# dotnetpower/infomesh

Measured on AMD Instinct MI355X. Metric: queries/sec (hybrid BM25+dense search, 1.25M docs), higher is better.
Workload: dtype bf16; 1 GPU; model=bge-small-en(random-init) encoder + BM25 CSR + cosine top-k, global_batch=128, seq_len=32, parallelism=shard1, mode=hybrid, docs_per_gpu=1250000, total_docs=1250000

## Files before the change

infomesh_amd/models/bert.py:

```python
from __future__ import annotations

from dataclasses import dataclass

import torch

from ..ops import kernels as K
from ..ops import reference as R


@dataclass(frozen=True)
class BertConfig:
    vocab_size: int
    hidden: int
    layers: int
    heads: int
    ffn: int
    max_pos: int = 512
    eps: float = 1e-12

    @property
    def head_dim(self) -> int:
        return self.hidden // self.heads


# ... 6 lines not shown

    def w(*shape, s=std):
        return torch.randn(*shape, generator=g) * s

    ws: dict[str, torch.Tensor] = {
        "embed.word": w(cfg.vocab_size, H),
        "embed.pos": w(cfg.max_pos, H),
        "embed.ln.g": torch.ones(H),
        "embed.ln.b": torch.zeros(H),
    }
    for i in range(cfg.layers):
        p = f"layer.{i}."
        ws[p + "qkv.w"] = w(3 * H, H)
        ws[p + "qkv.b"] = torch.zeros(3 * H)
        ws[p + "attn_out.w"] = w(H, H)
        ws[p + "attn_out.b"] = torch.zeros(H)
        ws[p + "ln1.g"] = torch.ones(H)
        ws[p + "ln1.b"] = torch.zeros(H)
        ws[p + "ffn_in.w"] = w(F, H)
        ws[p + "ffn_in.b"] = torch.zeros(F)
        ws[p + "ffn_out.w"] = w(H, F)
        ws[p + "ffn_out.b"] = torch.zeros(H)
        ws[p + "ln2.g"] = torch.ones(H)
        ws[p + "ln2.b"] = torch.zeros(H)
    out = {}
    for k, v in ws.items():
        t = v.to(device)
        out[k] = t if k.endswith(".b") and "ln" not in k else t.to(dtype)
        if "ln" in k:
            out[k] = t.to(dtype)
    return out


class BertEncoder:
    def __init__(self, cfg: BertConfig, weights: dict[str, torch.Tensor],
                 use_fused_attn: bool = True):
        self.cfg = cfg
        self.w = weights
        self.use_fused_attn = use_fused_attn and cfg.head_dim in (32, 64,
                                                                  96, 128)

    def forward(self, ids: torch.Tensor, lens: torch.Tensor) -> torch.Tensor:
        cfg, w = self.cfg, self.w
        B, S = ids.shape
        if S % 32 != 0:
            pad = 32 - S % 32
            ids = torch.nn.functional.pad(ids, (0, pad))
            S += pad
        H, nh, d = cfg.hidden, cfg.heads, cfg.head_dim
        pos_ids = torch.arange(S, device=ids.device, dtype=torch.int32)\
            .repeat(B)
        x = K.gather(w["embed.word"], ids.reshape(-1))
        x = K.add(x, K.gather(w["embed.pos"], pos_ids))
        x = K.layernorm(x, w["embed.ln.g"], w["embed.ln.b"], eps=cfg.eps)

        vl = lens.repeat_interleave(nh).contiguous()
        scale = d ** -0.5
        vl_b = lens.contiguous()
        for i in range(cfg.layers):
            p = f"layer.{i}."
            qkv = K.gemm_nt(x, w[p + "qkv.w"], bias=w[p + "qkv.b"])
            if self.use_fused_attn:
                qkv5 = qkv.view(B, S, 3, nh, d)
                qv = qkv5[:, :, 0].permute(0, 2, 1, 3)
                kv = qkv5[:, :, 1].permute(0, 2, 1, 3)
                vv = qkv5[:, :, 2].permute(0, 2, 1, 3)
                ctx = K.attn_fused(qv, kv, vv, valid_len=vl_b, scale=scale)
            else:
                q, k, vt = K.qkv_split(qkv, B, S, nh, nh, d)
                scores = K.gemm_nt(q, k, out_f32=True, alpha=scale)
                probs = K.softmax(scores, valid_len=vl)
                ctx = K.gemm_nt(probs, vt)
            merged = K.merge_heads(ctx, B, S, nh, d)
            attn = K.gemm_nt(merged, w[p + "attn_out.w"],
                             bias=w[p + "attn_out.b"])
            x = K.layernorm(attn, w[p + "ln1.g"], w[p + "ln1.b"],
                            residual=x, eps=cfg.eps)
            h = K.gemm_nt(x, w[p + "ffn_in.w"], bias=w[p + "ffn_in.b"],
                          act="gelu")
            o = K.gemm_nt(h, w[p + "ffn_out.w"], bias=w[p + "ffn_out.b"])
            x = K.layernorm(o, w[p + "ln2.g"], w[p + "ln2.b"],
                            residual=x, eps=cfg.eps)
        return x.view(B, S, H)

    def forward_reference(self, ids: torch.Tensor,
                          lens: torch.Tensor) -> torch.Tensor:
        cfg = self.cfg
        w = {k: v.float().cpu() for k, v in self.w.items()}
        B, S = ids.shape
        H, nh, d = cfg.hidden, cfg.heads, cfg.head_dim
        ids_l = ids.cpu().long()
        x = w["embed.word"][ids_l] + w["embed.pos"][:S].unsqueeze(0)
        x = R.layernorm(x, w["embed.ln.g"], w["embed.ln.b"], eps=cfg.eps)
        vl = lens.cpu().repeat_interleave(nh)
        for i in range(cfg.layers):
            p = f"layer.{i}."
            qkv = R.gemm_nt(x.view(B * S, H), w[p + "qkv.w"], w[p + "qkv.b"])
            qkv = qkv.view(B, S, 3, nh, d)
            q = qkv[:, :, 0].permute(0, 2, 1, 3).reshape(B * nh, S, d)
            k = qkv[:, :, 1].permute(0, 2, 1, 3).reshape(B * nh, S, d)
            v = qkv[:, :, 2].permute(0, 2, 1, 3).reshape(B * nh, S, d)
            scores = torch.matmul(q, k.transpose(1, 2)) * d ** -0.5
            probs = R.softmax(scores, valid_len=vl)
            ctx = torch.matmul(probs, v)
            merged = ctx.view(B, nh, S, d).permute(0, 2, 1, 3).reshape(B * S, H)
            attn = R.gemm_nt(merged, w[p + "attn_out.w"], w[p + "attn_out.b"])
            x = R.layernorm(attn, w[p + "ln1.g"], w[p + "ln1.b"],
                            residual=x.view(B * S, H), eps=cfg.eps)
            h = R.gemm_nt(x, w[p + "ffn_in.w"], w[p + "ffn_in.b"], act="gelu")
            o = R.gemm_nt(h, w[p + "ffn_out.w"], w[p + "ffn_out.b"])
            x = R.layernorm(o, w[p + "ln2.g"], w[p + "ln2.b"],
                            residual=x, eps=cfg.eps)
        return x.view(B, S, H)
```

infomesh_amd/models/encoder.py:

```python
from __future__ import annotations

import torch

from ..ops import kernels as K
from ..ops import reference as R
from .bert import BertConfig, BertEncoder, init_bert_weights
from .tokenizer import HashTokenizer

BGE_SMALL = BertConfig(vocab_size=30522, hidden=384, layers=12, heads=12,
                       ffn=1536, max_pos=512)

EMBED_DIM = BGE_SMALL.hidden


class EmbeddingEncoder:

    def __init__(self, device: str = "cuda", seed: int = 1234,
                 cfg: BertConfig = BGE_SMALL, max_len: int = 128,
                 use_graph: bool = True):
        self.cfg = cfg
        self.device = device
        self.max_len = max_len
        self.tokenizer = HashTokenizer(cfg.vocab_size)
        self.bert = BertEncoder(cfg, init_bert_weights(cfg, seed, device))
        from ..ops.graphs import GraphedCallable
        self._graphed = GraphedCallable(self._encode_impl, enabled=use_graph)

    def _encode_impl(self, ids: torch.Tensor,
                     lens: torch.Tensor) -> torch.Tensor:
        hidden = self.bert.forward(ids, lens)
        return K.pool(hidden, lens, mode="cls", l2=True)

    def encode_ids(self, ids: torch.Tensor, lens: torch.Tensor) -> torch.Tensor:
        return self._graphed(ids, lens)

    def encode_texts(self, texts: list[str]) -> torch.Tensor:
        ids_l, lens = self.tokenizer.encode_batch(texts, self.max_len)
        ids = torch.tensor(ids_l, dtype=torch.int32, device=self.device)
        lens_t = torch.tensor(lens, dtype=torch.int32, device=self.device)
        return self.encode_ids(ids, lens_t)

    def encode_ids_reference(self, ids: torch.Tensor,
                             lens: torch.Tensor) -> torch.Tensor:
        hidden = self.bert.forward_reference(ids, lens)
        return R.pool(hidden.bfloat16(), lens.cpu(), mode="cls", l2=True)
```

infomesh_amd/ops/_ext.py:

```python
from __future__ import annotations

import ctypes
from ctypes import c_float, c_int, c_long, c_void_p
from pathlib import Path

from ..errors import GpuExtensionMissing

_LIB: ctypes.CDLL | None = None
_LOAD_ERROR: str | None = None

_SIGNATURES: dict[str, list] = {
    "infomesh_gemm_bf16_nt": [c_void_p, c_void_p, c_void_p, c_void_p,
                              c_int, c_int, c_int, c_int,
                              c_long, c_long, c_long,
                              c_int, c_float, c_int, c_void_p],
    "infomesh_layernorm": [c_void_p, c_void_p, c_void_p, c_void_p,
                           c_void_p, c_void_p, c_long, c_int, c_float,
                           c_void_p],
    "infomesh_rmsnorm": [c_void_p, c_void_p, c_void_p, c_void_p,
                         c_void_p, c_long, c_int, c_float, c_void_p],
    "infomesh_softmax": [c_void_p, c_void_p, c_void_p, c_long, c_int,
                         c_int, c_int, c_float, c_void_p],
    "infomesh_bias_act": [c_void_p, c_void_p, c_long, c_int, c_int, c_void_p],
    "infomesh_silu_mul": [c_void_p, c_void_p, c_void_p, c_long, c_void_p],
    "infomesh_add": [c_void_p, c_void_p, c_void_p, c_long, c_void_p],
    "infomesh_rope": [c_void_p, c_void_p, c_void_p, c_void_p, c_long,
                      c_int, c_int, c_int, c_void_p],
    "infomesh_gather": [c_void_p, c_void_p, c_void_p, c_long, c_int,
                        c_float, c_void_p],
    "infomesh_pool": [c_void_p, c_void_p, c_void_p, c_int, c_int, c_int,
                      c_int, c_int, c_void_p],
    "infomesh_argmax": [c_void_p, c_void_p, c_long, c_int, c_void_p],
    "infomesh_topk": [c_void_p, c_void_p, c_void_p, c_void_p, c_int,
                      c_long, c_int, c_void_p, c_void_p],
    "infomesh_topk_masked": [c_void_p, c_void_p, c_void_p, c_void_p, c_int,
                             c_long, c_int, c_void_p, c_void_p, c_long,
                             c_void_p],
    "infomesh_filter_bitmask": [c_void_p, c_void_p, c_void_p, c_long,
                                c_int, c_void_p],
    "infomesh_filter_bitmask_sets": [c_void_p, c_void_p, c_void_p, c_void_p,
                                     c_void_p, c_long, c_int, c_void_p],
    "infomesh_term_bitmask": [c_void_p, c_long, c_void_p, c_void_p,
                              c_void_p, c_void_p, c_int, c_void_p, c_int,
                              c_long, c_long, c_long, c_long, c_void_p],
    "infomesh_term_block_docs": [],
    "infomesh_topk_workspace_u32": [c_int],
    "infomesh_topk_zero_u32": [c_int],
    "infomesh_bm25_block": [c_void_p, c_void_p, c_void_p, c_void_p,
                            c_void_p, c_void_p, c_void_p, c_void_p,
                            c_void_p, c_void_p, c_int, c_int, c_long,
                            c_long, c_long, c_int, c_float, c_float,
                            c_float, c_void_p],
    "infomesh_score_combine": [c_void_p, c_void_p, c_void_p, c_float,
                               c_float, c_long, c_void_p],
    "infomesh_simhash_fingerprint": [c_void_p, c_void_p, c_void_p, c_long,
                                     c_void_p],
    "infomesh_hamming_scan": [c_void_p, c_void_p, c_void_p, c_void_p,
                              c_void_p, c_void_p, c_int, c_long, c_int,
                              c_int, c_void_p],
    "infomesh_attn_decode": [c_void_p, c_void_p, c_void_p, c_void_p,
                             c_void_p, c_int, c_int, c_int, c_int, c_int,
                             c_float, c_void_p],
    "infomesh_attn_decode_split": [c_void_p, c_void_p, c_void_p, c_void_p,
                                   c_void_p, c_void_p, c_int, c_int, c_int,
                                   c_int, c_int, c_int, c_float, c_void_p],
    "infomesh_attn_fused": [c_void_p, c_void_p, c_void_p, c_void_p,
                            c_void_p, c_int, c_int, c_int, c_int, c_int,
                            c_int, c_long, c_long, c_long, c_long, c_long,
                            c_long, c_long, c_long, c_long,
                            c_int, c_float, c_void_p],
    "infomesh_kv_append": [c_void_p, c_void_p, c_void_p, c_void_p,
                           c_void_p, c_int, c_int, c_int, c_int, c_void_p],
    "infomesh_dense_scores": [c_void_p, c_void_p, c_void_p,
                              c_int, c_long, c_int, c_float, c_void_p],
    "infomesh_dense_scores_fp8": [c_void_p, c_void_p, c_void_p,
                                  c_int, c_long, c_int, c_float,
                                  c_void_p],
    "infomesh_gemm8_bf16_nt": [c_void_p, c_void_p, c_void_p, c_void_p,
                               c_int, c_int, c_int, c_int,
                               c_long, c_long, c_long,
                               c_int, c_float, c_int, c_void_p],
    "infomesh_gemv_bf16_nt": [c_void_p, c_void_p, c_void_p, c_void_p,
                              c_int, c_int, c_int, c_int,
                              c_long, c_long, c_long,
                              c_int, c_float, c_int, c_void_p],
    "infomesh_qkv_split": [c_void_p, c_void_p, c_void_p, c_void_p,
                           c_void_p, c_void_p, c_void_p,
                           c_int, c_int, c_int, c_int, c_int, c_int,
                           c_void_p],
    "infomesh_merge_heads": [c_void_p, c_void_p, c_int, c_int, c_int,
                             c_int, c_void_p],
    "infomesh_silu_mul_fused": [c_void_p, c_void_p, c_long, c_int,
                                c_void_p],
    "infomesh_gemm_tile": [c_int, c_int, c_int, c_int],
    "infomesh_gemm_bmax_width": [c_int, c_int, c_int, c_int],
    "infomesh_gemm_bf16_nt_bmax": [c_void_p, c_void_p, c_void_p, c_void_p,
                                   c_void_p, c_int, c_int, c_int, c_int,
                                   c_long, c_long, c_long,
                                   c_int, c_float, c_void_p],
    "infomesh_topk_pruned": [c_void_p, c_void_p, c_int, c_void_p, c_void_p,
                             c_void_p, c_int, c_long, c_int, c_void_p],
    "infomesh_topk_pruned_workspace_u32": [c_int, c_long, c_int, c_int],
    "infomesh_topk_pruned_zero_u32": [c_int],
# ... 13 lines not shown
    "infomesh_domtop_chunk_docs": [],
    "infomesh_domtop_lds_slots": [],
    "infomesh_domtop_k_max": [],
    "infomesh_domain_best": [c_void_p, c_void_p, c_void_p, c_void_p,
                             c_void_p, c_void_p, c_int, c_int, c_long,
                             c_long, c_int, c_int, c_int, c_int, c_void_p],
    "infomesh_collapse_select": [c_void_p, c_void_p, c_void_p, c_int, c_int,
                                 c_int, c_int, c_void_p],
    "infomesh_collapse_m_max": [],
    "infomesh_collapse_k_max": [],
    "infomesh_collapse_chunk_docs": [],
    "infomesh_collapse_lds_slots": [],
}

_RESTYPES = {"infomesh_topk_workspace_u32": c_long,
             "infomesh_collapse_m_max": c_int,
             "infomesh_collapse_k_max": c_int,
             "infomesh_collapse_chunk_docs": c_int,
             "infomesh_collapse_lds_slots": c_int,
             "infomesh_domtop_chunk_docs": c_int,
             "infomesh_domtop_lds_slots": c_int,
             "infomesh_domtop_k_max": c_int,
             "infomesh_facet_chunk_docs": c_int,
             "infomesh_facet_width": c_int,
             "infomesh_facet_slot": c_int,
             "infomesh_topk_zero_u32": c_long,
             "infomesh_topk_pruned_workspace_u32": c_long,
             "infomesh_topk_pruned_zero_u32": c_long,
             "infomesh_term_block_docs": c_int,
             "infomesh_gemm_bmax_width": c_int,
             "infomesh_gemm_bf16_nt_bmax": c_int,
             "infomesh_dense_scores": c_int,
             "infomesh_dense_scores_fp8": c_int,
             "infomesh_gemm_tile": c_int}


def _try_load() -> ctypes.CDLL | None:
    global _LOAD_ERROR
    so = Path(__file__).resolve().parent / "libinfomesh_hip.so"
    if not so.exists():
        _LOAD_ERROR = f"{so} not built"
        return None
    try:
        lib = ctypes.CDLL(str(so))
    except OSError as e:
        _LOAD_ERROR = str(e)
        return None
    for name, argtypes in _SIGNATURES.items():
        fn = getattr(lib, name)
        fn.argtypes = argtypes
        fn.restype = _RESTYPES.get(name)
    import os
    if os.environ.get("INFOMESH_SYNC_DEBUG"):
        return _SyncDebugLib(lib)
    return lib


class _SyncDebugLib:

    def __init__(self, real: ctypes.CDLL):
        self._real = real

    def __getattr__(self, name: str):
        fn = getattr(self._real, name)
        if not name.startswith("infomesh_"):
            return fn

# ... 34 lines not shown
```

infomesh_amd/ops/csrc/attn_fused.hip:

```cpp
#include "common.h"

#define QTILE 64
#define KTILE 64
#define VPAD 72

struct TensorView {
  const bf16* ptr;
  long bs, hs, rs;
};

namespace {

template <int D>
__global__ __launch_bounds__(256) void attn_fused_kernel(
    TensorView Q, TensorView K, TensorView V,
    const int* __restrict__ valid_len,
    bf16* __restrict__ O, int nhq, int nhk,
    int Sq, int Sk, int causal, float scale) {
  __shared__ bf16 k_lds[KTILE][D];
  __shared__ bf16 vt_lds[D][VPAD];
  __shared__ bf16 p_lds[4][16][KTILE];
  const int g = blockIdx.y;
  const int q0 = blockIdx.x * QTILE;
  const int lane = threadIdx.x & 63;
  const int wid = threadIdx.x >> 6;
  const int b = g / nhq, hq = g % nhq;
  const int hk = hq / (nhq / nhk);
  const int limit_all = valid_len ? min(Sk, valid_len[b]) : Sk;

  const bf16* Qg = Q.ptr + (long)b * Q.bs + (long)hq * Q.hs;
  const bf16* Kg = K.ptr + (long)b * K.bs + (long)hk * K.hs;
  const bf16* Vg = V.ptr + (long)b * V.bs + (long)hk * V.hs;

  const int qrow_f = lane & 15;
  const int kslice = lane >> 4;
  bf16x8 qfrag[D / 32];
  {
    const int qr = min(q0 + wid * 16 + qrow_f, Sq - 1);
#pragma unroll
    for (int f = 0; f < D / 32; ++f)
      qfrag[f] = *reinterpret_cast<const bf16x8*>(
          Qg + (long)qr * Q.rs + f * 32 + kslice * 8);
  }

  f32x4 o_acc[D / 16];
#pragma unroll
  for (int f = 0; f < D / 16; ++f) o_acc[f] = f32x4{0.f, 0.f, 0.f, 0.f};
  float m_run[4], l_run[4];
#pragma unroll
  for (int r = 0; r < 4; ++r) { m_run[r] = -INFINITY; l_run[r] = 0.f; }
  const int crow0 = (lane >> 4) * 4;
  const int ccol = lane & 15;

  int kv_limit = limit_all;
  if (causal) {
    const int max_q = min(q0 + QTILE - 1, Sq - 1);
    kv_limit = min(kv_limit, max_q + (Sk - Sq) + 1);
  }

  for (int kv0 = 0; kv0 < kv_limit; kv0 += KTILE) {
    {
      const int perrow = D / 8;
      for (int t = threadIdx.x; t < KTILE * perrow; t += 256) {
        const int key = t / perrow, dc = (t % perrow) * 8;
        const int src = min(kv0 + key, Sk - 1);
        *reinterpret_cast<bf16x8*>(&k_lds[key][dc]) =
            *reinterpret_cast<const bf16x8*>(Kg + (long)src * K.rs + dc);
        const bf16x8 vv = *reinterpret_cast<const bf16x8*>(
            Vg + (long)src * V.rs + dc);
#pragma unroll
        for (int j = 0; j < 8; ++j) vt_lds[dc + j][key] = vv[j];
      }
    }
    __syncthreads();

    f32x4 s_chunk[KTILE / 16];
#pragma unroll
    for (int kc = 0; kc < KTILE / 16; ++kc) {
      f32x4 acc = f32x4{0.f, 0.f, 0.f, 0.f};
#pragma unroll
      for (int f = 0; f < D / 32; ++f) {
        const bf16x8 kf = *reinterpret_cast<const bf16x8*>(
            &k_lds[kc * 16 + qrow_f][f * 32 + kslice * 8]);
        acc = __builtin_amdgcn_mfma_f32_16x16x32_bf16(
            qfrag[f], kf, acc, 0, 0, 0);
      }
      s_chunk[kc] = acc;
    }

    float tile_max[4];
#pragma unroll
    for (int r = 0; r < 4; ++r) tile_max[r] = -INFINITY;
#pragma unroll
    for (int kc = 0; kc < KTILE / 16; ++kc) {
      const int key = kv0 + kc * 16 + ccol;
      const bool key_ok = key < limit_all;
// ... 37 lines not shown
    for (int r = 0; r < 4; ++r) {
#pragma unroll
      for (int off = 1; off < 16; off <<= 1)
        row_sum[r] += __shfl_xor(row_sum[r], off, 64);
      l_run[r] = l_run[r] * alpha[r] + row_sum[r];
    }

#pragma unroll
    for (int f = 0; f < D / 16; ++f)
#pragma unroll
      for (int r = 0; r < 4; ++r) o_acc[f][r] *= alpha[r];

#pragma unroll
    for (int kc = 0; kc < KTILE / 16; ++kc)
#pragma unroll
      for (int r = 0; r < 4; ++r)
        p_lds[wid][crow0 + r][kc * 16 + ccol] = f2bf(s_chunk[kc][r]);

#pragma unroll
    for (int f = 0; f < D / 16; ++f) {
#pragma unroll
      for (int ks = 0; ks < KTILE / 32; ++ks) {
        const bf16x8 pf = *reinterpret_cast<const bf16x8*>(
            &p_lds[wid][qrow_f][ks * 32 + kslice * 8]);
        const bf16x8 vf = *reinterpret_cast<const bf16x8*>(
            &vt_lds[f * 16 + qrow_f][ks * 32 + kslice * 8]);
        o_acc[f] = __builtin_amdgcn_mfma_f32_16x16x32_bf16(
            pf, vf, o_acc[f], 0, 0, 0);
      }
    }
    __syncthreads();
  }

#pragma unroll
  for (int f = 0; f < D / 16; ++f) {
#pragma unroll
    for (int r = 0; r < 4; ++r) {
      const int qrow = q0 + wid * 16 + crow0 + r;
      if (qrow >= Sq) continue;
      const float inv = l_run[r] > 0.f ? 1.0f / l_run[r] : 0.f;
      O[(long)g * Sq * D + (long)qrow * D + f * 16 + ccol] =
          f2bf(o_acc[f][r] * inv);
    }
  }
}

}

extern "C" void infomesh_attn_fused(
    const void* Q, const void* K, const void* V, const void* valid_len,
    void* O, int B, int nhq, int nhk, int Sq, int Sk, int D,
    long qb, long qh, long qr, long kb, long kh, long kr,
    long vb, long vh, long vr,
    int causal, float scale, void* stream) {
  auto s = reinterpret_cast<hipStream_t>(stream);
  dim3 grid((Sq + QTILE - 1) / QTILE, B * nhq), block(256);
  TensorView qv{(const bf16*)Q, qb, qh, qr};
  TensorView kv{(const bf16*)K, kb, kh, kr};
  TensorView vv{(const bf16*)V, vb, vh, vr};
#define CASE(DV)                                                          \
  case DV:                                                                \
    hipLaunchKernelGGL(attn_fused_kernel<DV>, grid, block, 0, s,          \
                       qv, kv, vv, (const int*)valid_len, (bf16*)O,       \
                       nhq, nhk, Sq, Sk, causal, scale);                  \
    break;
  switch (D) {
    CASE(32) CASE(64) CASE(96) CASE(128)
    default:
      break;
  }
#undef CASE
}
```

infomesh_amd/ops/csrc/norms.hip:

```cpp
#include "common.h"

namespace {

template <bool RMS, bool RESIDUAL>
__global__ __launch_bounds__(256) void norm_kernel(
    const bf16* __restrict__ x, const bf16* __restrict__ res,
    bf16* __restrict__ out, bf16* __restrict__ res_out,
    const bf16* __restrict__ gamma, const bf16* __restrict__ beta,
    int H, float eps) {
  __shared__ float scratch[16];
  const long row = blockIdx.x;
  const bf16* xr = x + row * H;
  const bf16* rr = RESIDUAL ? res + row * H : nullptr;

  constexpr int MAXV = 8;
  f32x4 keep[2 * MAXV];
  const int nvec = H / 8;
  float sum = 0.f, sumsq = 0.f;
  for (int v = threadIdx.x, it = 0; v < nvec; v += blockDim.x, ++it) {
    bf16x8 xv = *reinterpret_cast<const bf16x8*>(xr + v * 8);
    float f[8];
#pragma unroll
    for (int j = 0; j < 8; ++j) f[j] = bf2f(xv[j]);
    if (RESIDUAL) {
      bf16x8 rv = *reinterpret_cast<const bf16x8*>(rr + v * 8);
#pragma unroll
      for (int j = 0; j < 8; ++j) f[j] += bf2f(rv[j]);
      if (res_out) {
        bf16x8 ov;
#pragma unroll
        for (int j = 0; j < 8; ++j) ov[j] = f2bf(f[j]);
        *reinterpret_cast<bf16x8*>(res_out + row * H + v * 8) = ov;
      }
    }
#pragma unroll
    for (int j = 0; j < 8; ++j) { sum += f[j]; sumsq += f[j] * f[j]; }
    if (it < MAXV) {
      keep[2 * it] = f32x4{f[0], f[1], f[2], f[3]};
      keep[2 * it + 1] = f32x4{f[4], f[5], f[6], f[7]};
    }
  }
  float mean = 0.f;
  if (!RMS) {
    mean = block_reduce_sum(sum, scratch) / H;
    __syncthreads();
  }
// ... 3 lines not shown
  for (int v = threadIdx.x, it = 0; v < nvec; v += blockDim.x, ++it) {
    float f[8];
    if (it < MAXV) {
#pragma unroll
      for (int j = 0; j < 4; ++j) f[j] = keep[2 * it][j];
#pragma unroll
      for (int j = 0; j < 4; ++j) f[4 + j] = keep[2 * it + 1][j];
    } else {
      bf16x8 xv = *reinterpret_cast<const bf16x8*>(xr + v * 8);
#pragma unroll
      for (int j = 0; j < 8; ++j) f[j] = bf2f(xv[j]);
      if (RESIDUAL) {
        bf16x8 rv = *reinterpret_cast<const bf16x8*>(rr + v * 8);
#pragma unroll
        for (int j = 0; j < 8; ++j) f[j] += bf2f(rv[j]);
      }
    }
    bf16x8 gv = *reinterpret_cast<const bf16x8*>(gamma + v * 8);
    bf16x8 ov;
    if (!RMS && beta) {
      bf16x8 bv = *reinterpret_cast<const bf16x8*>(beta + v * 8);
#pragma unroll
      for (int j = 0; j < 8; ++j)
        ov[j] = f2bf((f[j] - mean) * inv * bf2f(gv[j]) + bf2f(bv[j]));
    } else {
#pragma unroll
      for (int j = 0; j < 8; ++j)
        ov[j] = f2bf((f[j] - (RMS ? 0.f : mean)) * inv * bf2f(gv[j]));
    }
    *reinterpret_cast<bf16x8*>(out + row * H + v * 8) = ov;
  }
}

template <bool RMS, bool RESIDUAL>
__global__ __launch_bounds__(256) void norm_rowwave_kernel(
    const bf16* __restrict__ x, const bf16* __restrict__ res,
    bf16* __restrict__ out, bf16* __restrict__ res_out,
    const bf16* __restrict__ gamma, const bf16* __restrict__ beta,
    long rows, int H, float eps) {
  const long row = (long)blockIdx.x * 4 + (threadIdx.x >> 6);
  if (row >= rows) return;
  const int lane = threadIdx.x & 63;
  const bf16* xr = x + row * H;
  const bf16* rr = RESIDUAL ? res + row * H : nullptr;
  const int nvec = H / 8;
  float f[8 * 4];
  float sum = 0.f, sumsq = 0.f;
  int it = 0;
  for (int v = lane; v < nvec; v += 64, ++it) {
    bf16x8 xv = *reinterpret_cast<const bf16x8*>(xr + v * 8);
#pragma unroll
    for (int j = 0; j < 8; ++j) f[it * 8 + j] = bf2f(xv[j]);
    if (RESIDUAL) {
      bf16x8 rv = *reinterpret_cast<const bf16x8*>(rr + v * 8);
#pragma unroll
      for (int j = 0; j < 8; ++j) f[it * 8 + j] += bf2f(rv[j]);
      if (res_out) {
        bf16x8 ov;
#pragma unroll
        for (int j = 0; j < 8; ++j) ov[j] = f2bf(f[it * 8 + j]);
        *reinterpret_cast<bf16x8*>(res_out + row * H + v * 8) = ov;
      }
    }
#pragma unroll
    for (int j = 0; j < 8; ++j) {
      sum += f[it * 8 + j];
      sumsq += f[it * 8 + j] * f[it * 8 + j];
    }
  }
  float mean = 0.f;
  if (!RMS) mean = wave_reduce_sum(sum) / H;
  const float ms = wave_reduce_sum(sumsq) / H;
  const float inv = rsqrtf((RMS ? ms : ms - mean * mean) + eps);
  it = 0;
  for (int v = lane; v < nvec; v += 64, ++it) {
    bf16x8 gv = *reinterpret_cast<const bf16x8*>(gamma + v * 8);
    bf16x8 ov;
    if (!RMS && beta) {
      bf16x8 bv = *reinterpret_cast<const bf16x8*>(beta + v * 8);
#pragma unroll
      for (int j = 0; j < 8; ++j)
        ov[j] = f2bf((f[it * 8 + j] - mean) * inv * bf2f(gv[j])
                     + bf2f(bv[j]));
    } else {
#pragma unroll
      for (int j = 0; j < 8; ++j)
        ov[j] = f2bf((f[it * 8 + j] - (RMS ? 0.f : mean)) * inv
                     * bf2f(gv[j]));
    }
    *reinterpret_cast<bf16x8*>(out + row * H + v * 8) = ov;
  }
}

}

#define NORM_LAUNCH(RMS, RES, ...)                                        \
  do {                                                                    \
    if (H <= 2048) {                                                      \
      dim3 g((unsigned)((rows + 3) / 4));                                 \
      hipLaunchKernelGGL((norm_rowwave_kernel<RMS, RES>), g, dim3(256),   \
                         0, s, __VA_ARGS__, rows, H, eps);                \
    } else {                                                              \
      dim3 g((unsigned)rows);                                             \
      hipLaunchKernelGGL((norm_kernel<RMS, RES>), g, dim3(256), 0, s,     \
                         __VA_ARGS__, H, eps);                            \
    }                                                                     \
  } while (0)

extern "C" void infomesh_layernorm(
    const void* x, const void* residual, void* out, void* res_out,
    const void* gamma, const void* beta,
    long rows, int H, float eps, void* stream) {
  auto s = reinterpret_cast<hipStream_t>(stream);
  if (residual)
    NORM_LAUNCH(false, true, (const bf16*)x, (const bf16*)residual,
                (bf16*)out, (bf16*)res_out, (const bf16*)gamma,
                (const bf16*)beta);
  else
    NORM_LAUNCH(false, false, (const bf16*)x, nullptr, (bf16*)out,
                nullptr, (const bf16*)gamma, (const bf16*)beta);
}

extern "C" void infomesh_rmsnorm(
    const void* x, const void* residual, void* out, void* res_out,
    const void* gamma, long rows, int H, float eps, void* stream) {
  auto s = reinterpret_cast<hipStream_t>(stream);
  if (residual)
    NORM_LAUNCH(true, true, (const bf16*)x, (const bf16*)residual,
                (bf16*)out, (bf16*)res_out, (const bf16*)gamma, nullptr);
  else
    NORM_LAUNCH(true, false, (const bf16*)x, nullptr, (bf16*)out,
                nullptr, (const bf16*)gamma, nullptr);
}
```

infomesh_amd/ops/kernels.py:

```python
from __future__ import annotations

import torch

from . import _ext

ACT = {"none": 0, "gelu": 1, "silu": 2, "relu": 3, "tanh": 4}


def _ptr(t: torch.Tensor | None) -> int | None:
    return None if t is None else t.data_ptr()


def _check(t: torch.Tensor, dtype: torch.dtype, name: str) -> None:
    assert t.is_cuda, f"{name} must be on GPU"
    assert t.dtype == dtype, f"{name} must be {dtype}, got {t.dtype}"
    assert t.is_contiguous(), f"{name} must be contiguous"


def gemm_route(M: int, N: int, K: int, G: int) -> str:
    if M <= 16:
        return "gemv"
    if (M >= 4096 and N >= 512 and K % 64 == 0
            and ((M + 255) // 256) * ((N + 255) // 256) * max(G, 1) >= 224):
        return "gemm8"
# ... 89 lines not shown
    if out is None:
        out = torch.empty(M, N, device=a.device, dtype=torch.float32)
    rc = _ext.lib().infomesh_dense_scores(
        a.data_ptr(), b.data_ptr(), out.data_ptr(), M, N, K, alpha,
        _ext.stream_ptr())
    return out if rc == 0 else None


def dense_scores_fp8(a: torch.Tensor, b: torch.Tensor,
                     alpha: float = 1.0,
                     out: torch.Tensor | None = None
                     ) -> torch.Tensor | None:
    M, K = a.shape
    N = b.shape[0]
    assert a.dtype == torch.float8_e4m3fn and a.is_cuda and a.is_contiguous()
    assert b.dtype == torch.float8_e4m3fn and b.is_contiguous()
    if out is None:
        out = torch.empty(M, N, device=a.device, dtype=torch.float32)
    rc = _ext.lib().infomesh_dense_scores_fp8(
        a.data_ptr(), b.data_ptr(), out.data_ptr(), M, N, K, alpha,
        _ext.stream_ptr())
    return out if rc == 0 else None


def layernorm(x: torch.Tensor, gamma: torch.Tensor, beta: torch.Tensor,
              residual: torch.Tensor | None = None, eps: float = 1e-12,
              return_residual: bool = False):
    H = x.shape[-1]
    assert H % 8 == 0
    rows = x.numel() // H
    _check(x, torch.bfloat16, "x")
    out = torch.empty_like(x)
    res_out = None
    if residual is not None:
        assert residual.shape == x.shape
        if return_residual:
            res_out = torch.empty_like(x)
    _ext.lib().infomesh_layernorm(
        x.data_ptr(), _ptr(residual), out.data_ptr(), _ptr(res_out),
        gamma.data_ptr(), beta.data_ptr(), rows, H, eps, _ext.stream_ptr())
    return (out, res_out) if return_residual else out


def rmsnorm(x: torch.Tensor, gamma: torch.Tensor,
            residual: torch.Tensor | None = None, eps: float = 1e-5,
            return_residual: bool = False):
    H = x.shape[-1]
    assert H % 8 == 0
    rows = x.numel() // H
    _check(x, torch.bfloat16, "x")
    out = torch.empty_like(x)
    res_out = None
    if residual is not None and return_residual:
        res_out = torch.empty_like(x)
    _ext.lib().infomesh_rmsnorm(
        x.data_ptr(), _ptr(residual), out.data_ptr(), _ptr(res_out),
        gamma.data_ptr(), rows, H, eps, _ext.stream_ptr())
    if return_residual:
        return out, (res_out if res_out is not None else x)
    return out


def softmax(scores: torch.Tensor, scale: float = 1.0, causal: bool = False,
            valid_len: torch.Tensor | None = None,
            sq_dim: int | None = None) -> torch.Tensor:
    assert scores.dim() == 3
    _check(scores, torch.float32, "scores")
    G, Sq, Sk = scores.shape
    out = torch.empty_like(scores, dtype=torch.bfloat16)
    if valid_len is not None:
        _check(valid_len, torch.int32, "valid_len")
    _ext.lib().infomesh_softmax(
        scores.data_ptr(), out.data_ptr(), _ptr(valid_len),
        G, Sq, Sk, int(causal), scale, _ext.stream_ptr())
# ... 28 lines not shown
    _ext.lib().infomesh_add(a.data_ptr(), b.data_ptr(), out.data_ptr(),
                            a.numel(), _ext.stream_ptr())
    return out


def rope(x: torch.Tensor, cos_t: torch.Tensor, sin_t: torch.Tensor,
         pos: torch.Tensor, rot_dim: int | None = None) -> torch.Tensor:
    rows, H, D = x.shape
    rot = rot_dim or D
    _check(x, torch.bfloat16, "x")
    _check(pos, torch.int32, "pos")
    _ext.lib().infomesh_rope(
        x.data_ptr(), cos_t.data_ptr(), sin_t.data_ptr(), pos.data_ptr(),
        rows, H, D, rot, _ext.stream_ptr())
    return x


def gather(table: torch.Tensor, ids: torch.Tensor,
           scale: float = 1.0) -> torch.Tensor:
    _check(table, torch.bfloat16, "table")
    _check(ids, torch.int32, "ids")
    H = table.shape[1]
    out = torch.empty((ids.numel(), H), device=table.device,
                      dtype=torch.bfloat16)
    _ext.lib().infomesh_gather(table.data_ptr(), ids.data_ptr(),
                               out.data_ptr(), ids.numel(), H, scale,
                               _ext.stream_ptr())
    return out


def pool(x: torch.Tensor, lens: torch.Tensor | None = None,
         mode: str = "cls", l2: bool = True) -> torch.Tensor:
    B, S, H = x.shape
    _check(x, torch.bfloat16, "x")
    out = torch.empty((B, H), device=x.device, dtype=torch.float32)
    _ext.lib().infomesh_pool(
        x.data_ptr(), _ptr(lens), out.data_ptr(), B, S, H,
        {"cls": 0, "mean": 1}[mode], int(l2), _ext.stream_ptr())
    return out


def argmax(logits: torch.Tensor) -> torch.Tensor:
    rows, V = logits.shape
    _check(logits, torch.float32, "logits")
    out = torch.empty((rows,), device=logits.device, dtype=torch.int32)
    _ext.lib().infomesh_argmax(logits.data_ptr(), out.data_ptr(), rows, V,
                               _ext.stream_ptr())
    return out


class TopK:

    def __init__(self, device: torch.device | str = "cuda"):
        self.device = torch.device(device)
        self._ws: torch.Tensor | None = None

    def __call__(self, scores: torch.Tensor, k: int,
                 ext_hist1: torch.Tensor | None = None,
                 mask: torch.Tensor | None = None,
                 row_pred: torch.Tensor | None = None
                 ) -> tuple[torch.Tensor, torch.Tensor]:
        assert scores.dim() == 2
        _check(scores, torch.float32, "scores")
        B, N = scores.shape
        assert 1 <= k <= 1024
        assert (mask is None) == (row_pred is None), \
            "mask and row_pred go together"
# ... 482 lines not shown
                                      _ext.stream_ptr())
    return out


def simhash_fingerprint(offsets: torch.Tensor,
                        hashes: torch.Tensor) -> torch.Tensor:
    ndocs = offsets.numel() - 1
    out = torch.empty(ndocs, device=offsets.device, dtype=torch.int64)
    _ext.lib().infomesh_simhash_fingerprint(
        offsets.data_ptr(), hashes.data_ptr(), out.data_ptr(), ndocs,
        _ext.stream_ptr())
    return out


def hamming_scan(queries: torch.Tensor, table: torch.Tensor,
                 radius: int = 3, cap: int = 65536
                 ) -> tuple[torch.Tensor, torch.Tensor, torch.Tensor]:
    M, N = queries.numel(), table.numel()
    dev = table.device
    out_q = torch.empty(cap, device=dev, dtype=torch.int32)
    out_n = torch.empty(cap, device=dev, dtype=torch.int32)
    out_d = torch.empty(cap, device=dev, dtype=torch.int32)
    cnt = torch.zeros(1, device=dev, dtype=torch.int32)
    _ext.lib().infomesh_hamming_scan(
        queries.data_ptr(), table.data_ptr(), out_q.data_ptr(),
        out_n.data_ptr(), out_d.data_ptr(), cnt.data_ptr(), M, N, radius,
        cap, _ext.stream_ptr())
    n = min(int(cnt.item()), cap)
    return out_q[:n], out_n[:n], out_d[:n]


def attn_fused(q: torch.Tensor, k: torch.Tensor, v: torch.Tensor,
               valid_len: torch.Tensor | None = None,
               causal: bool = False, scale: float | None = None
               ) -> torch.Tensor:
    assert q.dim() == 4 and k.dim() == 4 and v.dim() == 4
    B, nh, Sq, d = q.shape
    _, nhk, Sk, dk = k.shape
    assert d == dk and d in (32, 64, 96, 128) and nh % nhk == 0
    for t in (q, k, v):
        assert t.dtype == torch.bfloat16 and t.stride(3) == 1
    if scale is None:
        scale = d ** -0.5
    out = torch.empty(B * nh, Sq, d, device=q.device, dtype=torch.bfloat16)
    if valid_len is not None:
        _check(valid_len, torch.int32, "valid_len")
        assert valid_len.numel() == B
    _ext.lib().infomesh_attn_fused(
        q.data_ptr(), k.data_ptr(), v.data_ptr(), _ptr(valid_len),
        out.data_ptr(), B, nh, nhk, Sq, Sk, d,
        q.stride(0), q.stride(1), q.stride(2),
        k.stride(0), k.stride(1), k.stride(2),
        v.stride(0), v.stride(1), v.stride(2),
        int(causal), scale, _ext.stream_ptr())
    return out


def attn_decode(q: torch.Tensor, k_cache: torch.Tensor,
                v_cache: torch.Tensor, lens: torch.Tensor,
                scale: float) -> torch.Tensor:
    import math
    B, H, D = q.shape
    _, Hkv, Smax, _ = k_cache.shape
    _check(q, torch.bfloat16, "q")
    assert D % 8 == 0 and D <= 128
    out = torch.empty_like(q)
    nc_min = max(1, math.ceil(Smax / 2048))
    nc = max(nc_min, min(64, math.ceil(512 / max(1, B * H))))
    if nc <= 1:
        _ext.lib().infomesh_attn_decode(
            q.data_ptr(), k_cache.data_ptr(), v_cache.data_ptr(),
            lens.data_ptr(), out.data_ptr(), B, H, Hkv, Smax, D, scale,
            _ext.stream_ptr())
    else:
        part = torch.empty(B, H, nc, D + 2, device=q.device,
                           dtype=torch.float32)
        _ext.lib().infomesh_attn_decode_split(
            q.data_ptr(), k_cache.data_ptr(), v_cache.data_ptr(),
            lens.data_ptr(), part.data_ptr(), out.data_ptr(),
            B, H, Hkv, Smax, D, nc, scale, _ext.stream_ptr())
    return out


def qkv_split(qkv: torch.Tensor, B: int, S: int, nh: int, nkv: int,
              d: int, cos_t: torch.Tensor | None = None,
              sin_t: torch.Tensor | None = None,
              pos: torch.Tensor | None = None,
              rot: int | None = None, want_vt: bool = True
# ... 43 lines not shown
```

Baseline: 43540 queries/s.

## Fuse embed+layernorm, write attention into merged layout, shrink tile, trim CLS-only tail

Four changes to the encoder. A single kernel now does the embedding gather, position add and layernorm. Attention writes straight into the merged-heads layout, so the merge_heads kernel goes away. A 32x32 attention tile is added for short sequences, which cuts wasted work when seq_len is 32. In the last layer only the CLS query row is computed through attention, the output projection and the FFN, with the layernorm reading a strided residual. Together these remove launches and memory traffic and skip rows that pooling never reads. In exchange there are more kernel variants, and the tail path depends on the GEMM tile choice matching for B versus B*S rows.

```diff
diff --git a/infomesh_amd/models/bert.py b/infomesh_amd/models/bert.py
--- a/infomesh_amd/models/bert.py
+++ b/infomesh_amd/models/bert.py
@@ -62,56 +62,107 @@
     return out
 
 
+FAST_ITEMS = frozenset({"merge", "short", "tail", "embed"})
+
+
+def cls_tail_gemms(H: int, F: int) -> tuple[tuple[int, int], ...]:
+    return ((H, H), (F, H), (H, F))
+
+
+def cls_tail_routes_match(B: int, rows: int, H: int, F: int) -> bool:
+    return all(K.gemm_route(B, N, Kd, 1) == "gemm"
+               and K.gemm_route(rows, N, Kd, 1) == "gemm"
+               for N, Kd in cls_tail_gemms(H, F))
+
+
+def cls_tail_same_kernel(B: int, rows: int, H: int, F: int) -> bool:
+    return cls_tail_routes_match(B, rows, H, F) and all(
+        K.gemm_tile(B, N, Kd, 1) == K.gemm_tile(rows, N, Kd, 1)
+        for N, Kd in cls_tail_gemms(H, F))
+
+
 class BertEncoder:
     def __init__(self, cfg: BertConfig, weights: dict[str, torch.Tensor],
-                 use_fused_attn: bool = True):
+                 use_fused_attn: bool = True,
+                 fast_path: bool | frozenset[str] | set[str] = True):
         self.cfg = cfg
         self.w = weights
         self.use_fused_attn = use_fused_attn and cfg.head_dim in (32, 64,
                                                                   96, 128)
+        if isinstance(fast_path, bool):
+            fast_path = FAST_ITEMS if fast_path else frozenset()
+        self.fast = frozenset(fast_path)
+        assert self.fast <= FAST_ITEMS, f"unknown items {self.fast - FAST_ITEMS}"
+        if not self.use_fused_attn:
+            self.fast -= {"merge", "short", "tail"}
 
-    def forward(self, ids: torch.Tensor, lens: torch.Tensor) -> torch.Tensor:
+    def forward(self, ids: torch.Tensor, lens: torch.Tensor,
+                cls_only: bool = False) -> torch.Tensor:
         cfg, w = self.cfg, self.w
+        fast = self.fast
         B, S = ids.shape
         if S % 32 != 0:
             pad = 32 - S % 32
             ids = torch.nn.functional.pad(ids, (0, pad))
             S += pad
         H, nh, d = cfg.hidden, cfg.heads, cfg.head_dim
-        pos_ids = torch.arange(S, device=ids.device, dtype=torch.int32)\
-            .repeat(B)
-        x = K.gather(w["embed.word"], ids.reshape(-1))
-        x = K.add(x, K.gather(w["embed.pos"], pos_ids))
-        x = K.layernorm(x, w["embed.ln.g"], w["embed.ln.b"], eps=cfg.eps)
+        if "embed" in fast:
+            x = K.embed_layernorm(w["embed.word"], w["embed.pos"],
+                                  ids.reshape(-1), S, w["embed.ln.g"],
+                                  w["embed.ln.b"], eps=cfg.eps)
+        else:
+            pos_ids = torch.arange(S, device=ids.device, dtype=torch.int32)\
+                .repeat(B)
+            x = K.gather(w["embed.word"], ids.reshape(-1))
+            x = K.add(x, K.gather(w["embed.pos"], pos_ids))
+            x = K.layernorm(x, w["embed.ln.g"], w["embed.ln.b"], eps=cfg.eps)
 
-        vl = lens.repeat_interleave(nh).contiguous()
         scale = d ** -0.5
         vl_b = lens.contiguous()
+        if not self.use_fused_attn:
+            vl = lens.repeat_interleave(nh).contiguous()
+        variant = 0 if "short" in fast else 1
+        tail = (cls_only and "tail" in fast
+                and cls_tail_same_kernel(B, B * S, H, cfg.ffn))
         for i in range(cfg.layers):
             p = f"layer.{i}."
             qkv = K.gemm_nt(x, w[p + "qkv.w"], bias=w[p + "qkv.b"])
+            Sq = 1 if tail and i == cfg.layers - 1 else S
             if self.use_fused_attn:
                 qkv5 = qkv.view(B, S, 3, nh, d)
-                qv = qkv5[:, :, 0].permute(0, 2, 1, 3)
+                qv = qkv5[:, :Sq, 0].permute(0, 2, 1, 3)
                 kv = qkv5[:, :, 1].permute(0, 2, 1, 3)
                 vv = qkv5[:, :, 2].permute(0, 2, 1, 3)
-                ctx = K.attn_fused(qv, kv, vv, valid_len=vl_b, scale=scale)
+                if "merge" in fast:
+                    merged = torch.empty(B * Sq, H, device=x.device,
+                                         dtype=torch.bfloat16)
+                    K.attn_fused(qv, kv, vv, valid_len=vl_b, scale=scale,
+                                 out=merged.view(B, Sq, nh, d)
+                                 .permute(0, 2, 1, 3), variant=variant)
+                else:
+                    ctx = K.attn_fused(qv, kv, vv, valid_len=vl_b,
+                                       scale=scale, variant=variant)
+                    merged = K.merge_heads(ctx, B, Sq, nh, d)
             else:
                 q, k, vt = K.qkv_split(qkv, B, S, nh, nh, d)
                 scores = K.gemm_nt(q, k, out_f32=True, alpha=scale)
                 probs = K.softmax(scores, valid_len=vl)
                 ctx = K.gemm_nt(probs, vt)
-            merged = K.merge_heads(ctx, B, S, nh, d)
+                merged = K.merge_heads(ctx, B, S, nh, d)
             attn = K.gemm_nt(merged, w[p + "attn_out.w"],
                              bias=w[p + "attn_out.b"])
+            res = x.view(B, S, H)[:, 0] if Sq != S else x
             x = K.layernorm(attn, w[p + "ln1.g"], w[p + "ln1.b"],
-                            residual=x, eps=cfg.eps)
+                            residual=res, eps=cfg.eps)
             h = K.gemm_nt(x, w[p + "ffn_in.w"], bias=w[p + "ffn_in.b"],
                           act="gelu")
             o = K.gemm_nt(h, w[p + "ffn_out.w"], bias=w[p + "ffn_out.b"])
             x = K.layernorm(o, w[p + "ln2.g"], w[p + "ln2.b"],
                             residual=x, eps=cfg.eps)
-        return x.view(B, S, H)
+        if tail:
+            return x.view(B, 1, H)
+        x = x.view(B, S, H)
+        return x[:, :1] if cls_only else x
 
     def forward_reference(self, ids: torch.Tensor,
                           lens: torch.Tensor) -> torch.Tensor:
diff --git a/infomesh_amd/models/encoder.py b/infomesh_amd/models/encoder.py
--- a/infomesh_amd/models/encoder.py
+++ b/infomesh_amd/models/encoder.py
@@ -17,18 +17,20 @@
 
     def __init__(self, device: str = "cuda", seed: int = 1234,
                  cfg: BertConfig = BGE_SMALL, max_len: int = 128,
-                 use_graph: bool = True):
+                 use_graph: bool = True,
+                 fast_path: bool | frozenset[str] | set[str] = True):
         self.cfg = cfg
         self.device = device
         self.max_len = max_len
         self.tokenizer = HashTokenizer(cfg.vocab_size)
-        self.bert = BertEncoder(cfg, init_bert_weights(cfg, seed, device))
+        self.bert = BertEncoder(cfg, init_bert_weights(cfg, seed, device),
+                                fast_path=fast_path)
         from ..ops.graphs import GraphedCallable
         self._graphed = GraphedCallable(self._encode_impl, enabled=use_graph)
 
     def _encode_impl(self, ids: torch.Tensor,
                      lens: torch.Tensor) -> torch.Tensor:
-        hidden = self.bert.forward(ids, lens)
+        hidden = self.bert.forward(ids, lens, cls_only=True)
         return K.pool(hidden, lens, mode="cls", l2=True)
 
     def encode_ids(self, ids: torch.Tensor, lens: torch.Tensor) -> torch.Tensor:
diff --git a/infomesh_amd/ops/_ext.py b/infomesh_amd/ops/_ext.py
--- a/infomesh_amd/ops/_ext.py
+++ b/infomesh_amd/ops/_ext.py
@@ -16,7 +16,10 @@
                               c_int, c_float, c_int, c_void_p],
     "infomesh_layernorm": [c_void_p, c_void_p, c_void_p, c_void_p,
                            c_void_p, c_void_p, c_long, c_int, c_float,
-                           c_void_p],
+                           c_long, c_void_p],
+    "infomesh_embed_layernorm": [c_void_p, c_void_p, c_void_p, c_void_p,
+                                 c_void_p, c_void_p, c_long, c_int, c_int,
+                                 c_float, c_void_p],
     "infomesh_rmsnorm": [c_void_p, c_void_p, c_void_p, c_void_p,
                          c_void_p, c_long, c_int, c_float, c_void_p],
     "infomesh_softmax": [c_void_p, c_void_p, c_void_p, c_long, c_int,
@@ -68,7 +71,8 @@
                             c_void_p, c_int, c_int, c_int, c_int, c_int,
                             c_int, c_long, c_long, c_long, c_long, c_long,
                             c_long, c_long, c_long, c_long,
-                            c_int, c_float, c_void_p],
+                            c_long, c_long, c_long,
+                            c_int, c_float, c_int, c_void_p],
     "infomesh_kv_append": [c_void_p, c_void_p, c_void_p, c_void_p,
                            c_void_p, c_int, c_int, c_int, c_int, c_void_p],
     "infomesh_dense_scores": [c_void_p, c_void_p, c_void_p,
@@ -148,7 +152,9 @@
              "infomesh_gemm_bf16_nt_bmax": c_int,
              "infomesh_dense_scores": c_int,
              "infomesh_dense_scores_fp8": c_int,
-             "infomesh_gemm_tile": c_int}
+             "infomesh_gemm_tile": c_int,
+             "infomesh_attn_fused": c_int,
+             "infomesh_embed_layernorm": c_int}
 
 
 def _try_load() -> ctypes.CDLL | None:
diff --git a/infomesh_amd/ops/csrc/attn_fused.hip b/infomesh_amd/ops/csrc/attn_fused.hip
--- a/infomesh_amd/ops/csrc/attn_fused.hip
+++ b/infomesh_amd/ops/csrc/attn_fused.hip
@@ -1,25 +1,28 @@
 #include "common.h"
-
-#define QTILE 64
-#define KTILE 64
-#define VPAD 72
 
 struct TensorView {
   const bf16* ptr;
   long bs, hs, rs;
 };
+struct OutView {
+  bf16* ptr;
+  long bs, hs, rs;
+};
 
 namespace {
 
-template <int D>
-__global__ __launch_bounds__(256) void attn_fused_kernel(
+template <int D, int QTILE, int KTILE>
+__global__ __launch_bounds__(QTILE * 4) void attn_fused_kernel(
     TensorView Q, TensorView K, TensorView V,
     const int* __restrict__ valid_len,
-    bf16* __restrict__ O, int nhq, int nhk,
+    OutView O, int nhq, int nhk,
     int Sq, int Sk, int causal, float scale) {
+  constexpr int NW = QTILE / 16;
+  constexpr int NT = NW * 64;
+  constexpr int VPAD = KTILE + 8;
   __shared__ bf16 k_lds[KTILE][D];
   __shared__ bf16 vt_lds[D][VPAD];
-  __shared__ bf16 p_lds[4][16][KTILE];
+  __shared__ bf16 p_lds[NW][16][KTILE];
   const int g = blockIdx.y;
   const int q0 = blockIdx.x * QTILE;
   const int lane = threadIdx.x & 63;
@@ -61,7 +64,7 @@
   for (int kv0 = 0; kv0 < kv_limit; kv0 += KTILE) {
     {
       const int perrow = D / 8;
-      for (int t = threadIdx.x; t < KTILE * perrow; t += 256) {
+      for (int t = threadIdx.x; t < KTILE * perrow; t += NT) {
         const int key = t / perrow, dc = (t % perrow) * 8;
         const int src = min(kv0 + key, Sk - 1);
         *reinterpret_cast<bf16x8*>(&k_lds[key][dc]) =
@@ -165,6 +168,7 @@
     __syncthreads();
   }
 
+  bf16* Og = O.ptr + (long)b * O.bs + (long)hq * O.hs;
 #pragma unroll
   for (int f = 0; f < D / 16; ++f) {
 #pragma unroll
@@ -172,30 +176,23 @@
       const int qrow = q0 + wid * 16 + crow0 + r;
       if (qrow >= Sq) continue;
       const float inv = l_run[r] > 0.f ? 1.0f / l_run[r] : 0.f;
-      O[(long)g * Sq * D + (long)qrow * D + f * 16 + ccol] =
-          f2bf(o_acc[f][r] * inv);
-    }
-  }
-}
-
-}
-
-extern "C" void infomesh_attn_fused(
-    const void* Q, const void* K, const void* V, const void* valid_len,
-    void* O, int B, int nhq, int nhk, int Sq, int Sk, int D,
-    long qb, long qh, long qr, long kb, long kh, long kr,
-    long vb, long vh, long vr,
-    int causal, float scale, void* stream) {
-  auto s = reinterpret_cast<hipStream_t>(stream);
-  dim3 grid((Sq + QTILE - 1) / QTILE, B * nhq), block(256);
-  TensorView qv{(const bf16*)Q, qb, qh, qr};
-  TensorView kv{(const bf16*)K, kb, kh, kr};
-  TensorView vv{(const bf16*)V, vb, vh, vr};
+      Og[(long)qrow * O.rs + f * 16 + ccol] = f2bf(o_acc[f][r] * inv);
+    }
+  }
+}
+
+constexpr int SHORT_TILE = 32;
+
+template <int QTILE, int KTILE>
+void launch_attn(int D, TensorView q, TensorView k, TensorView v,
+                 const int* valid_len, OutView o, int B, int nhq, int nhk,
+                 int Sq, int Sk, int causal, float scale, hipStream_t s) {
+  dim3 grid((Sq + QTILE - 1) / QTILE, B * nhq), block(QTILE * 4);
 #define CASE(DV)                                                          \
   case DV:                                                                \
-    hipLaunchKernelGGL(attn_fused_kernel<DV>, grid, block, 0, s,          \
-                       qv, kv, vv, (const int*)valid_len, (bf16*)O,       \
-                       nhq, nhk, Sq, Sk, causal, scale);                  \
+    hipLaunchKernelGGL((attn_fused_kernel<DV, QTILE, KTILE>), grid,       \
+                       block, 0, s, q, k, v, valid_len, o, nhq, nhk,      \
+                       Sq, Sk, causal, scale);                            \
     break;
   switch (D) {
     CASE(32) CASE(64) CASE(96) CASE(128)
@@ -204,3 +201,28 @@
   }
 #undef CASE
 }
+
+}
+
+extern "C" int infomesh_attn_fused(
+    const void* Q, const void* K, const void* V, const void* valid_len,
+    void* O, int B, int nhq, int nhk, int Sq, int Sk, int D,
+    long qb, long qh, long qr, long kb, long kh, long kr,
+    long vb, long vh, long vr, long ob, long oh, long orow,
+    int causal, float scale, int variant, void* stream) {
+  auto s = reinterpret_cast<hipStream_t>(stream);
+  const bool fits = Sq <= SHORT_TILE && Sk <= SHORT_TILE;
+  if (variant < 0 || variant > 2 || (variant == 2 && !fits)) return 1;
+  TensorView qv{(const bf16*)Q, qb, qh, qr};
+  TensorView kv{(const bf16*)K, kb, kh, kr};
+  TensorView vv{(const bf16*)V, vb, vh, vr};
+  OutView ov{(bf16*)O, ob, oh, orow};
+  if (variant == 2 || (variant == 0 && fits))
+    launch_attn<SHORT_TILE, SHORT_TILE>(D, qv, kv, vv, (const int*)valid_len,
+                                        ov, B, nhq, nhk, Sq, Sk, causal,
+                                        scale, s);
+  else
+    launch_attn<64, 64>(D, qv, kv, vv, (const int*)valid_len, ov, B, nhq,
+                        nhk, Sq, Sk, causal, scale, s);
+  return 0;
+}
diff --git a/infomesh_amd/ops/csrc/norms.hip b/infomesh_amd/ops/csrc/norms.hip
--- a/infomesh_amd/ops/csrc/norms.hip
+++ b/infomesh_amd/ops/csrc/norms.hip
@@ -7,11 +7,11 @@
     const bf16* __restrict__ x, const bf16* __restrict__ res,
     bf16* __restrict__ out, bf16* __restrict__ res_out,
     const bf16* __restrict__ gamma, const bf16* __restrict__ beta,
-    int H, float eps) {
+    int H, float eps, long res_stride) {
   __shared__ float scratch[16];
   const long row = blockIdx.x;
   const bf16* xr = x + row * H;
-  const bf16* rr = RESIDUAL ? res + row * H : nullptr;
+  const bf16* rr = RESIDUAL ? res + row * res_stride : nullptr;
 
   constexpr int MAXV = 8;
   f32x4 keep[2 * MAXV];
@@ -81,17 +81,20 @@
   }
 }
 
-template <bool RMS, bool RESIDUAL>
+template <bool RMS, bool RESIDUAL, bool EMBED = false>
 __global__ __launch_bounds__(256) void norm_rowwave_kernel(
     const bf16* __restrict__ x, const bf16* __restrict__ res,
     bf16* __restrict__ out, bf16* __restrict__ res_out,
     const bf16* __restrict__ gamma, const bf16* __restrict__ beta,
-    long rows, int H, float eps) {
+    long rows, int H, float eps, long res_stride,
+    const int* __restrict__ ids, int S) {
   const long row = (long)blockIdx.x * 4 + (threadIdx.x >> 6);
   if (row >= rows) return;
   const int lane = threadIdx.x & 63;
-  const bf16* xr = x + row * H;
-  const bf16* rr = RESIDUAL ? res + row * H : nullptr;
+  const bf16* xr = x + (EMBED ? (long)ids[row] : row) * H;
+  const bf16* rr = EMBED      ? res + (row % S) * H
+                   : RESIDUAL ? res + row * res_stride
+                              : nullptr;
   const int nvec = H / 8;
   float f[8 * 4];
   float sum = 0.f, sumsq = 0.f;
@@ -100,7 +103,12 @@
     bf16x8 xv = *reinterpret_cast<const bf16x8*>(xr + v * 8);
 #pragma unroll
     for (int j = 0; j < 8; ++j) f[it * 8 + j] = bf2f(xv[j]);
-    if (RESIDUAL) {
+    if (EMBED) {
+      bf16x8 rv = *reinterpret_cast<const bf16x8*>(rr + v * 8);
+#pragma unroll
+      for (int j = 0; j < 8; ++j)
+        f[it * 8 + j] = bf2f(f2bf(f[it * 8 + j] + bf2f(rv[j])));
+    } else if (RESIDUAL) {
       bf16x8 rv = *reinterpret_cast<const bf16x8*>(rr + v * 8);
 #pragma unroll
       for (int j = 0; j < 8; ++j) f[it * 8 + j] += bf2f(rv[j]);
@@ -148,18 +156,19 @@
     if (H <= 2048) {                                                      \
       dim3 g((unsigned)((rows + 3) / 4));                                 \
       hipLaunchKernelGGL((norm_rowwave_kernel<RMS, RES>), g, dim3(256),   \
-                         0, s, __VA_ARGS__, rows, H, eps);                \
+                         0, s, __VA_ARGS__, rows, H, eps, res_stride,     \
+                         nullptr, 1);                                     \
     } else {                                                              \
       dim3 g((unsigned)rows);                                             \
       hipLaunchKernelGGL((norm_kernel<RMS, RES>), g, dim3(256), 0, s,     \
-                         __VA_ARGS__, H, eps);                            \
+                         __VA_ARGS__, H, eps, res_stride);                \
     }                                                                     \
   } while (0)
 
 extern "C" void infomesh_layernorm(
     const void* x, const void* residual, void* out, void* res_out,
     const void* gamma, const void* beta,
-    long rows, int H, float eps, void* stream) {
+    long rows, int H, float eps, long res_stride, void* stream) {
   auto s = reinterpret_cast<hipStream_t>(stream);
   if (residual)
     NORM_LAUNCH(false, true, (const bf16*)x, (const bf16*)residual,
@@ -174,6 +183,7 @@
     const void* x, const void* residual, void* out, void* res_out,
     const void* gamma, long rows, int H, float eps, void* stream) {
   auto s = reinterpret_cast<hipStream_t>(stream);
+  const long res_stride = H;
   if (residual)
     NORM_LAUNCH(true, true, (const bf16*)x, (const bf16*)residual,
                 (bf16*)out, (bf16*)res_out, (const bf16*)gamma, nullptr);
@@ -181,3 +191,17 @@
     NORM_LAUNCH(true, false, (const bf16*)x, nullptr, (bf16*)out,
                 nullptr, (const bf16*)gamma, nullptr);
 }
+
+extern "C" int infomesh_embed_layernorm(
+    const void* word, const void* pos, const void* ids, void* out,
+    const void* gamma, const void* beta,
+    long rows, int S, int H, float eps, void* stream) {
+  auto s = reinterpret_cast<hipStream_t>(stream);
+  if (H > 2048 || H % 8 != 0 || S < 1) return 1;
+  dim3 g((unsigned)((rows + 3) / 4));
+  hipLaunchKernelGGL((norm_rowwave_kernel<false, false, true>), g, dim3(256),
+                     0, s, (const bf16*)word, (const bf16*)pos, (bf16*)out,
+                     nullptr, (const bf16*)gamma, (const bf16*)beta, rows, H,
+                     eps, (long)H, (const int*)ids, S);
+  return 0;
+}
diff --git a/infomesh_amd/ops/kernels.py b/infomesh_amd/ops/kernels.py
--- a/infomesh_amd/ops/kernels.py
+++ b/infomesh_amd/ops/kernels.py
@@ -145,14 +145,44 @@
     _check(x, torch.bfloat16, "x")
     out = torch.empty_like(x)
     res_out = None
+    res_stride = H
     if residual is not None:
         assert residual.shape == x.shape
+        assert residual.dtype == torch.bfloat16 and residual.is_cuda
+        if not residual.is_contiguous():
+            assert residual.dim() == 2 and residual.stride(1) == 1 \
+                and residual.stride(0) >= H and residual.stride(0) % 8 == 0 \
+                and residual.storage_offset() % 8 == 0, \
+                "residual must be contiguous or a 2-D row-strided view"
+            res_stride = residual.stride(0)
         if return_residual:
             res_out = torch.empty_like(x)
     _ext.lib().infomesh_layernorm(
         x.data_ptr(), _ptr(residual), out.data_ptr(), _ptr(res_out),
-        gamma.data_ptr(), beta.data_ptr(), rows, H, eps, _ext.stream_ptr())
+        gamma.data_ptr(), beta.data_ptr(), rows, H, eps, res_stride,
+        _ext.stream_ptr())
     return (out, res_out) if return_residual else out
+
+
+def embed_layernorm(word: torch.Tensor, pos: torch.Tensor,
+                    ids: torch.Tensor, S: int, gamma: torch.Tensor,
+                    beta: torch.Tensor, eps: float = 1e-12) -> torch.Tensor:
+    _check(word, torch.bfloat16, "word")
+    _check(pos, torch.bfloat16, "pos")
+    _check(ids, torch.int32, "ids")
+    _check(gamma, torch.bfloat16, "gamma")
+    _check(beta, torch.bfloat16, "beta")
+    H = word.shape[1]
+    assert pos.shape[1] == H and gamma.numel() == H and beta.numel() == H
+    assert 1 <= S <= pos.shape[0] and ids.numel() % S == 0
+    out = torch.empty((ids.numel(), H), device=word.device,
+                      dtype=torch.bfloat16)
+    rc = _ext.lib().infomesh_embed_layernorm(
+        word.data_ptr(), pos.data_ptr(), ids.data_ptr(), out.data_ptr(),
+        gamma.data_ptr(), beta.data_ptr(), ids.numel(), S, H, eps,
+        _ext.stream_ptr())
+    assert rc == 0, f"embed_layernorm does not cover H={H}"
+    return out
 
 
 def rmsnorm(x: torch.Tensor, gamma: torch.Tensor,
@@ -247,7 +277,12 @@
 def pool(x: torch.Tensor, lens: torch.Tensor | None = None,
          mode: str = "cls", l2: bool = True) -> torch.Tensor:
     B, S, H = x.shape
-    _check(x, torch.bfloat16, "x")
+    if mode == "cls" and S == 1 and not x.is_contiguous():
+        assert x.is_cuda and x.dtype == torch.bfloat16
+        assert x.stride(2) == 1 and x.stride(0) % H == 0 and x.stride(0) > 0
+        S = x.stride(0) // H
+    else:
+        _check(x, torch.bfloat16, "x")
     out = torch.empty((B, H), device=x.device, dtype=torch.float32)
     _ext.lib().infomesh_pool(
         x.data_ptr(), _ptr(lens), out.data_ptr(), B, S, H,
@@ -796,8 +831,9 @@
 
 def attn_fused(q: torch.Tensor, k: torch.Tensor, v: torch.Tensor,
                valid_len: torch.Tensor | None = None,
-               causal: bool = False, scale: float | None = None
-               ) -> torch.Tensor:
+               causal: bool = False, scale: float | None = None,
+               out: torch.Tensor | None = None, variant: int = 0
+               ) -> torch.Tensor | None:
     assert q.dim() == 4 and k.dim() == 4 and v.dim() == 4
     B, nh, Sq, d = q.shape
     _, nhk, Sk, dk = k.shape
@@ -806,18 +842,28 @@
         assert t.dtype == torch.bfloat16 and t.stride(3) == 1
     if scale is None:
         scale = d ** -0.5
-    out = torch.empty(B * nh, Sq, d, device=q.device, dtype=torch.bfloat16)
+    assert k.shape[0] == B and v.shape == k.shape and Sq >= 1 and Sk >= 1
+    if out is None:
+        ret = torch.empty(B * nh, Sq, d, device=q.device,
+                          dtype=torch.bfloat16)
+        ostr = (nh * Sq * d, Sq * d, d)
+        optr = ret.data_ptr()
+    else:
+        assert out.shape == (B, nh, Sq, d) and out.is_cuda
+        assert out.dtype == torch.bfloat16 and out.stride(3) == 1
+        ret, ostr, optr = out, out.stride()[:3], out.data_ptr()
     if valid_len is not None:
         _check(valid_len, torch.int32, "valid_len")
         assert valid_len.numel() == B
-    _ext.lib().infomesh_attn_fused(
+    rc = _ext.lib().infomesh_attn_fused(
         q.data_ptr(), k.data_ptr(), v.data_ptr(), _ptr(valid_len),
-        out.data_ptr(), B, nh, nhk, Sq, Sk, d,
+        optr, B, nh, nhk, Sq, Sk, d,
         q.stride(0), q.stride(1), q.stride(2),
         k.stride(0), k.stride(1), k.stride(2),
         v.stride(0), v.stride(1), v.stride(2),
-        int(causal), scale, _ext.stream_ptr())
-    return out
+        ostr[0], ostr[1], ostr[2],
+        int(causal), scale, variant, _ext.stream_ptr())
+    return ret if rc == 0 else None
 
 
 def attn_decode(q: torch.Tensor, k_cache: torch.Tensor,
```

Measured after the change: 44640 queries/s, median of 6. +2.5%, better.
